# k-flouris/cmf

Measured on AMD Instinct MI355X. Metric: log-density evals/sec (JtJ-cholesky path), MNIST D=784 d=64 bs=512, higher is better.
Workload: dtype f32 (3x3 tangent convs as bf16x3 split MFMA, fp32 accumulate); 1 GPU; C3: MNIST-shaped (1,28,28) uint8-range + U[0,1) noise, non-square flow d=64, cholesky J^T J log-det + g_ij off-diagonal L1 + reconstruction, eval/no_grad; per_gpu_batch=512, global_batch=512, D=784, latent_dimension=64, parallelism=dp1

## Files before the change

### cmf_amd/_lib.py

```python
import ctypes as C
import os
import threading

_HERE = os.path.dirname(os.path.abspath(__file__))
LIB_PATH = os.path.join(_HERE, "libcmf_amd.so")

F_NONE, F_RELU, F_TANH, F_RAW, F_SELF_RELU, F_RELU_BITS = 0, 1, 2, 3, 4, 5
O_NONE, O_TANH, O_STANH = 0, 1, 2

_fp = C.c_void_p
_ll = C.c_longlong
_i = C.c_int
_f = C.c_float
_d = C.c_double


class ConvTangentArgs(C.Structure):
    _fields_ = [("x", _fp), ("x_np", _ll), ("x_ci", _ll), ("x_px", _ll),
                ("f", _fp), ("f_np", _ll), ("f_ci", _ll), ("f_px", _ll), ("fmode", _i),
                ("w", _fp),
                ("y", _fp), ("y_np", _ll), ("y_co", _ll), ("y_px", _ll),
                ("r", _fp), ("r_np", _ll), ("r_co", _ll), ("r_px", _ll),
                ("np", _i), ("cin", _i), ("cout", _i), ("H", _i), ("W", _i), ("nc", _i), ("taps", _i),
                ("bias", _fp), ("f_group", _i), ("x_sl", _ll), ("y_sl", _ll), ("r_sl", _ll),
                ("fo", _fp), ("fo_np", _ll), ("fo_co", _ll), ("fo_px", _ll), ("fomode", _i),
                ("mask_out", _fp), ("mask_np", _ll), ("amax_in", _fp), ("amax_out", _fp), ("live", _i),
                ("ymask", _fp), ("ymask_np", _ll)]


class ConvPrimalArgs(C.Structure):
    _fields_ = [("x", _fp), ("x_b", _ll), ("x_c", _ll), ("x_px", _ll),
                ("f", _fp), ("f_c", _ll), ("f_px", _ll), ("imode", _i),
                ("w", _fp), ("bias", _fp), ("sw", _fp), ("sb", _fp),
                ("y", _fp), ("y_b", _ll), ("y_c", _ll), ("y_px", _ll),
                ("g", _fp),
                ("r", _fp), ("r_b", _ll), ("r_c", _ll), ("r_px", _ll),
                ("omode", _i),
                ("B", _i), ("cin", _i), ("cout", _i), ("H", _i), ("W", _i), ("taps", _i)]


MLP_MAX_LAYERS = 8
WGRAD_MAX_BATCH = 16


class MlpCouplerArgs(C.Structure):
    _fields_ = [("z", _fp), ("z_b", _ll), ("t", _fp), ("t_f", _ll), ("w", _fp),
                ("zi", _fp), ("si", _fp), ("ti", _fp), ("n_mod", _i),
                ("B", _i), ("cin", _i), ("chan_off", _i), ("chan_step", _i), ("n_layers", _i),
                ("width", _i * (MLP_MAX_LAYERS + 1)), ("w_off", _ll * MLP_MAX_LAYERS), ("decode", _i), ("lj", _fp), ("ncols", _i)]


SIGNATURES = {
    "cmf_version": (C.c_char_p, []),
    "cmf_pack_weight": (_i, [_fp, _fp, _i, _i, _i, _i, C.POINTER(_ll), _fp]),
    "cmf_pack_weights_batched": (_i, [_fp, _i, _fp]),
    "cmf_conv_tangent": (_i, [C.POINTER(ConvTangentArgs), _fp]),
    "cmf_pack_weight_bf16x3": (_i, [_fp, _fp, _i, _i, C.POINTER(_ll), _fp]),
    "cmf_pack_weight_bf16x3_t": (_i, [_fp, _fp, _i, _i, _i, C.POINTER(_ll), _fp]),
    "cmf_conv_tangent_bf16x3": (_i, [C.POINTER(ConvTangentArgs), _fp]),
    "cmf_pack_weight_f16x3": (_i, [_fp, _fp, _i, _i, _i, C.POINTER(_ll), _fp]),
    "cmf_conv_tangent_f16x3": (_i, [C.POINTER(ConvTangentArgs), _fp]),
    "cmf_conv_tangent_f16x3_item": (_i, [C.POINTER(ConvTangentArgs), _i, _fp]),
    "cmf_absmax": (_i, [_fp, _ll, _fp, _fp]),
    "cmf_conv_tangent_wgrad_ws": (_ll, [C.POINTER(ConvTangentArgs)]),
    "cmf_conv_tangent_wgrad": (_i, [C.POINTER(ConvTangentArgs), _fp, _fp, _fp, _ll, _fp]),
    "cmf_conv_tangent_wgrad_bf16x3": (_i, [C.POINTER(ConvTangentArgs), _fp, _fp, _fp, _ll, _fp]),
    "cmf_conv_tangent_wgrad_bf16x3_batched": (_i, [C.POINTER(ConvTangentArgs), _i, C.POINTER(_fp), C.POINTER(_fp), C.POINTER(_fp), _fp, _ll, _fp]),
    "cmf_primal_regroup": (_i, [_fp, _fp, _i, _ll, _i, _fp]),
    "cmf_conv_primal": (_i, [C.POINTER(ConvPrimalArgs), _fp]),
    "cmf_acl_primal": (_i, [_fp, _ll, _fp, _ll, _fp, _fp, _fp, _i, _i, _i, _fp, _fp]),
    "cmf_acl_tangent": (_i, [_fp, _ll, _ll, _fp, _ll, _ll, _i, _fp, _ll, _fp, _ll, _fp, _fp, _fp, _fp, _i, _i, _fp]),
    "cmf_acl_cotangent": (_i, [_fp, _ll, _ll, _fp, _ll, _ll, _i, _fp, _ll, _fp, _ll, _fp, _fp, _fp, _fp, _i, _i, _fp]),
    "cmf_acl_primal_backward": (_i, [_fp, _ll, _fp, _ll, _fp, _ll, _fp, _fp, _fp, _fp, _i, _i, _i, _fp, _fp]),
    "cmf_acl_cross_terms": (_i, [_fp, _ll, _ll, _fp, _ll, _ll, _fp, _ll, _ll, _i, _fp, _ll, _fp, _ll, _fp, _fp, _fp, _fp, _i, _i,
                            _fp, _fp, _fp, _fp]),
    "cmf_gather_primal": (_i, [_fp, _ll, _fp, _ll, _fp, _i, _i, _fp]),
    "cmf_gather_tangent": (_i, [_fp, _ll, _ll, _fp, _ll, _ll, _fp, _i, _i, _i, _fp]),
    "cmf_seed_tangent": (_i, [_fp, _ll, _ll, _fp, _i, _i, _fp, _i, _i, _i, _fp]),
    "cmf_gram_cholesky": (_i, [_fp, _ll, _ll, _i, _i, _i, _i, _fp, _fp, _fp, _fp, _fp, _fp, _fp]),
    "cmf_cholesky_retry": (_i, [_fp, _i, _i, _i, _f, _fp, _fp, _fp, _fp, _fp]),
# ... 131 lines not shown
```

### cmf_amd/csrc/common.h

```cpp
#pragma once
#include <hip/hip_runtime.h>
#include "cmf_amd.h"

typedef float f32x4 __attribute__((ext_vector_type(4)));

#define CMF_LAUNCH_CHECK()                         \
  do {                                             \
    hipError_t e_ = hipGetLastError();             \
    if (e_ != hipSuccess) return (int)e_;          \
  } while (0)

hipError_t cmf_set_dynamic_lds(const void* fn, int bytes);
int cmf_device_cus();

static inline int cmf_ceil_div(long long a, long long b) { return (int)((a + b - 1) / b); }

__device__ __forceinline__ float wave_sum(float v) {
#pragma unroll
  for (int o = 32; o > 0; o >>= 1) v += __shfl_xor(v, o, 64);
  return v;
}

__device__ __forceinline__ float block_sum(float v, float* red) {
  v = wave_sum(v);
  const int w = threadIdx.x >> 6, nw = (blockDim.x + 63) >> 6;
  __syncthreads();
  if ((threadIdx.x & 63) == 0) red[w] = v;
  __syncthreads();
  float t = 0.f;
  for (int i = 0; i < nw; ++i) t += red[i];
  return t;
}

int cmf_wide_gram_cholesky(const float* t, long long t_b, long long t_r, int n_rows, int d, int B, float* jtj, float* logdet,
                           float* l1_off, float* l1_diag, int* info, int* fail, hipStream_t s);
int cmf_wide_cholesky_retry(float* jtj, int d, int B, int attempt, float eps, float* logdet, float* l1_diag, int* info, int* fail,
                            hipStream_t s);
int cmf_wide_gram_backward(const float* t, long long t_b, long long t_r, int n_rows, int nc, int d, int B, const float* jtj,
                           const float* g_logdet, const float* g_l1off, const float* g_l1diag, float* dt, long long dt_b,
                           long long dt_r, float* ws, hipStream_t s);
int cmf_wide_gram_backward_matrix(const float* t, long long t_b, long long t_r, int n_rows, int nc, int d, int B, const float* m,
                                  float* dt, long long dt_b, long long dt_r, hipStream_t s);
int cmf_wide_hutch_cg(const float* jtj, const float* eps, int d, int S, int B, int max_iter, int min_iter, float tol, float* u,
                      float* w, float* val, int* iters, hipStream_t s);
int cmf_wide_hutch_cotangent(const float* u, const float* eps, const float* w, int d, int S, int B, const float* g_val,
                             const float* g_off, const float* g_diag, float* M, hipStream_t s);
```

### cmf_amd/csrc/conv_tangent_bf16x3.hip

```cpp
#include <cstdlib>
#include <type_traits>
#include "common.h"

#ifdef CMF_DBG_STAMP
__device__ unsigned long long cmf_dbg_stamps[3][64][4];
extern "C" int cmf_debug_read_stamps(void* out) {
  return (int)hipMemcpyFromSymbol(out, HIP_SYMBOL(cmf_dbg_stamps), sizeof(cmf_dbg_stamps));
}
#define STAMP(role, g, k)                                                                        \
  do {                                                                                            \
    if (blockIdx.x == 0 && (g) < 64 && lane == 0 && wave == ((role) == 1 ? 4 : 0)) {                   \
      unsigned long long t_;                                                                      \
      asm volatile("s_memtime %0\n\ts_waitcnt lgkmcnt(0)" : "=s"(t_)::"memory");                  \
      cmf_dbg_stamps[role][g][k] = t_;                                                            \
    }                                                                                             \
  } while (0)
__device__ unsigned long long cmf_dbg_wg_span[1024][2];
extern "C" int cmf_debug_read_wg_span(void* out) {
  return (int)hipMemcpyFromSymbol(out, HIP_SYMBOL(cmf_dbg_wg_span), sizeof(cmf_dbg_wg_span));
}
#define SPAN(k)                                                                                   \
  do {                                                                                            \
    if (lane == 0 && wave == 0 && blockIdx.x < 1024) {                                            \
      unsigned long long t_;                                                                      \
// ... 1027 lines not shown
}

template <int PXW>
int launch_cot(const cmf_conv_tangent_args& a, hipStream_t s) {
  if (a.ymask) return a.fmode == CMF_F_RELU ? launch<4, PXW, 6>(a, s) : launch<4, PXW, 7>(a, s);
  if (a.fmode == CMF_F_SELF_RELU) return (a.cout > 32) ? launch<4, PXW, 2>(a, s) : launch<2, PXW, 2>(a, s);
  if (a.fmode == CMF_F_RELU) return (a.cout > 32) ? launch<4, PXW, 1>(a, s) : launch<2, PXW, 1>(a, s);
  if (a.fmode == CMF_F_RELU_BITS) return (a.cout > 32) ? launch<4, PXW, 3>(a, s) : launch<2, PXW, 3>(a, s);
  if (a.fmode == CMF_F_NONE && a.fomode == CMF_F_RELU_BITS && a.r) {
    return launch<4, PXW, 5>(a, s);
  }
  if (a.fmode == CMF_F_NONE) return (a.cout > 32) ? launch<4, PXW, 4>(a, s) : launch<2, PXW, 4>(a, s);
  return (a.cout > 32) ? launch<4, PXW, 0>(a, s) : launch<2, PXW, 0>(a, s);
}

inline bool fits_int(long long v) { return v >= 0 && v < (1LL << 29); }

}

extern "C" int cmf_pack_weight_bf16x3_t(const float* w, void* out, int cout, int cin, int transpose, long long* out_bytes, void* stream);
extern "C" int cmf_pack_weight_bf16x3(const float* w, void* out, int cout, int cin, long long* out_bytes, void* stream) {
  return cmf_pack_weight_bf16x3_t(w, out, cout, cin, 0, out_bytes, stream);
}
extern "C" int cmf_pack_weight_bf16x3_t(const float* w, void* out, int cout, int cin, int transpose, long long* out_bytes, void* stream) {
  if (cout <= 0 || cin <= 0 || cin % 8) return CMF_EINVAL;
  const long long total = (long long)((cout + 63) / 64) * (cin / 8) * 2 * 3 * 4 * 4 * 16 * 8;
  if (out_bytes) *out_bytes = total * 2;
  if (!out) return 0;
  if (!w) return CMF_EINVAL;
  hipLaunchKernelGGL(pack_weight_bf16x3_kernel, dim3((unsigned)((total + 255) / 256)), dim3(256), 0, (hipStream_t)stream,
                     w, (unsigned short*)out, cout, cin, total, transpose ? 1 : 0, 0);
  CMF_LAUNCH_CHECK();
  return 0;
}

extern "C" int cmf_pack_weight_f16x3(const float* w, void* out, int cout, int cin, int transpose, long long* out_bytes, void* stream) {
  if (cout <= 0 || cin <= 0 || cin % 8) return CMF_EINVAL;
  const long long total = (long long)((cout + 63) / 64) * (cin / 8) * 2 * 3 * 4 * 4 * 16 * 8;
  if (out_bytes) *out_bytes = total * 2 + 16;
  if (!out) return 0;
  if (!w || (uintptr_t)out % 16) return CMF_EINVAL;
  hipLaunchKernelGGL(pack_f16_scale_kernel, dim3(1), dim3(1024), 0, (hipStream_t)stream, w, (long long)cout * cin * 9,
                     reinterpret_cast<float*>((unsigned short*)out + total));
  CMF_LAUNCH_CHECK();
  hipLaunchKernelGGL(pack_weight_bf16x3_kernel, dim3((unsigned)((total + 255) / 256)), dim3(256), 0, (hipStream_t)stream,
                     w, (unsigned short*)out, cout, cin, total, transpose ? 1 : 0, 1);
  CMF_LAUNCH_CHECK();
  return 0;
}

extern "C" int cmf_conv_tangent_bf16x3(const cmf_conv_tangent_args* ap, void* stream) {
  if (!ap) return CMF_EINVAL;
  const cmf_conv_tangent_args& a = *ap;
  if (!a.x || !a.w || !a.y || a.np <= 0 || a.cin <= 0 || a.cout <= 0 || a.H <= 0 || a.W <= 0) return CMF_EINVAL;
  if (a.taps != 9 || a.cin % 32 || a.nc <= 0 || a.nc % 16) return CMF_EINVAL;
  if (a.fmode < CMF_F_NONE || a.fmode > CMF_F_RELU_BITS) return CMF_EINVAL;
  if (a.fmode != CMF_F_SELF_RELU && a.fmode != CMF_F_NONE && !a.f) return CMF_EINVAL;
  if (a.mask_out) return CMF_EINVAL;
  if (a.fo) {
    const bool inplace = a.r == a.y && a.r_np == a.y_np && a.r_co == a.y_co && a.r_px == a.y_px && a.r_sl == a.y_sl;
    if (a.fmode != CMF_F_NONE || a.fomode != CMF_F_RELU_BITS || (a.r && !inplace) || a.cout % 64) return CMF_EINVAL;
    if (a.r && a.bias) return CMF_EINVAL;
    if (a.fo_np % 4 || (uintptr_t)a.fo % 4 || a.fo_np < (long long)a.H * a.W * (a.cout / 8)) return CMF_EINVAL;
  }
  if (a.fmode == CMF_F_RELU_BITS && a.f_np < (long long)a.H * a.W * (a.cin / 8)) return CMF_EINVAL;
  if (a.ymask) {
    if ((a.fmode != CMF_F_RELU && a.fmode != CMF_F_RELU_BITS) || a.cout % 64 || a.live || a.fo || a.r || a.bias) return CMF_EINVAL;
    if (a.ymask_np % 4 || (uintptr_t)a.ymask % 4 || a.ymask_np < (long long)a.H * a.W * (a.cout / 8)) return CMF_EINVAL;
  }
  if ((a.x_np | a.x_ci | a.x_px | a.x_sl | a.y_sl | a.r_sl) % 4 || ((uintptr_t)a.x % 16) || ((uintptr_t)a.w % 16)) return CMF_EINVAL;
  if ((a.y_np | a.y_co | a.y_px) % 4 || ((uintptr_t)a.y % 16)) return CMF_EINVAL;
  if (a.r && ((a.r_np | a.r_co | a.r_px) % 4 || ((uintptr_t)a.r % 16))) return CMF_EINVAL;
  const long long HW = (long long)a.H * a.W;
  if (!fits_int((a.cin + 8) * a.x_ci + HW * a.x_px + a.nc) || !fits_int((a.cin + 8) * a.f_ci + HW * a.f_px) ||
      !fits_int((a.cout + 64) * a.y_co + HW * a.y_px + a.nc + 64) ||
      (a.r && !fits_int((a.cout + 64) * a.r_co + HW * a.r_px + a.nc)) ||
      HW > (1 << 24))
    return CMF_ERANGE;
  hipStream_t s = (hipStream_t)stream;
  const bool t14 = a.W % 14 == 0 && a.H % 2 == 0, t8 = a.W % 8 == 0 && a.H % 4 == 0;
  if (!(t14 || t8) || !(a.cout % 64 == 0 || a.cout == 32)) return CMF_EINVAL;
  if (a.bias && a.cout > 64) return CMF_EINVAL;
  if (a.live) {
    if (a.live < 0 || a.live > 2 || (a.fmode != CMF_F_RELU && a.fmode != CMF_F_RELU_BITS) || a.fo || a.bias || a.cout % 64 || a.W % 2)
      return CMF_EINVAL;
    if (a.fmode == CMF_F_RELU) return t14 ? launch<4, 7, 1, false, false, true>(a, s) : launch<4, 4, 1, false, false, true>(a, s);
    return t14 ? launch<4, 7, 3, false, false, true>(a, s) : launch<4, 4, 3, false, false, true>(a, s);
  }
  if (a.fmode == CMF_F_NONE && !a.fo) {
    cmf_conv_tangent_args b = a;
    b.fo = a.x;
    b.fo_np = 0;
    b.fomode = CMF_F_NONE;
    return t14 ? launch_cot<7>(b, s) : launch_cot<4>(b, s);
  }
  return t14 ? launch_cot<7>(a, s) : launch_cot<4>(a, s);
}

extern "C" int cmf_conv_tangent_f16x3(const cmf_conv_tangent_args* ap, void* stream) {
  return cmf_conv_tangent_f16x3_item(ap, 0, stream);
}

extern "C" int cmf_conv_tangent_f16x3_item(const cmf_conv_tangent_args* ap, int item_channels, void* stream) {
  if (!ap || (item_channels != 0 && item_channels != 32 && item_channels != 64)) return CMF_EINVAL;
  const cmf_conv_tangent_args& a = *ap;
  if (!a.x || !a.w || !a.y || a.np <= 0 || a.cin <= 0 || a.cout <= 0 || a.H <= 0 || a.W <= 0) return CMF_EINVAL;
// ... 34 lines not shown
```

### cmf_amd/engine.py

```python
import ctypes as C
import threading

import numpy as np
import torch
import torch.nn as nn

from . import _lib
from ._lib import (F_NONE, F_RELU, F_TANH, F_RAW, F_SELF_RELU, F_RELU_BITS, O_NONE, O_TANH, O_STANH, ConvPrimalArgs,
                   ConvTangentArgs)


def _stream():
    return C.c_void_p(torch.cuda.current_stream().cuda_stream)


def _p(t):
    return None if t is None else C.c_void_p(t.data_ptr())


def require_gpu(t, what="input"):
    if not t.is_cuda:
        raise RuntimeError(f"cmf_amd: {what} is on {t.device}; the log-density path runs only through the HIP "
                           "kernels on an AMD GPU (there is no CPU fallback)")
    if t.dtype != torch.float32:
# ... 247 lines not shown
                continue
            if not isinstance(w, nn.Parameter):
                continue
            todo.append((key, w, ver, out, taps))
        if not todo:
            return
        desc = np.dtype([("w", "<u8"), ("out", "<u8"), ("total", "<i8"), ("cout", "<i4"), ("cin", "<i4"), ("taps", "<i4"),
                         ("transpose", "<i4"), ("kind", "<i4"), ("reserved", "<i4")])
        sig = tuple((key, w.data_ptr(), out.data_ptr()) for key, w, ver, out, taps in todo)
        cached = self._tables.get(device)
        if cached is not None and cached[0] == sig:
            table = cached[1]
        else:
            arr = np.zeros(len(todo), dtype=desc)
            for i, (key, w, ver, out, taps) in enumerate(todo):
                _, transpose, bf16x3 = key
                cout, cin = int(w.shape[0]), int(w.shape[1])
                if bf16x3 and transpose:
                    cout, cin = cin, cout
                total = out.numel() * out.element_size()
                total = (total - 16) // 2 if bf16x3 == 2 else total // (2 if bf16x3 else 4)
                arr[i] = (w.data_ptr(), out.data_ptr(), total, cout, cin, taps, int(transpose), int(bf16x3), 0)
            table = torch.from_numpy(arr.view(np.uint8).copy()).to(device)
            self._tables[device] = (sig, table)
        _lib.check(_lib.load().cmf_pack_weights_batched(_p(table), len(todo), _stream()), "cmf_pack_weights_batched")
        order = self._mark()
        for key, w, ver, out, taps in todo:
            self._store[key] = (self._store[key][0], ver[:4] + (self.generation,), out, taps, order)


PACKS = _PackCache()




def conv_primal(x_ptr_t, x_off, x_b, x_c, x_px, weight, taps, bias, y, y_b, y_c, y_px, B, cin, cout, H, W,
                imode=F_NONE, mask=None, f_c=0, f_px=0, omode=O_NONE, sw=None, sb=None, g=None, res=None):
    lib = _lib.load()
    a = ConvPrimalArgs()
    a.x = C.c_void_p(x_ptr_t.data_ptr() + 4 * int(x_off)); a.x_b, a.x_c, a.x_px = int(x_b), int(x_c), int(x_px)
    a.f = _p(mask); a.f_c, a.f_px = int(f_c), int(f_px); a.imode = imode
    a.w = _p(PACKS.get(weight, taps)); a.bias = _p(bias); a.sw = _p(sw); a.sb = _p(sb)
    a.y = _p(y); a.y_b, a.y_c, a.y_px = int(y_b), int(y_c), int(y_px)
    a.g = _p(g)
    a.r = _p(res); a.r_b, a.r_c, a.r_px = int(y_b), int(y_c), int(y_px)
    a.omode = omode
    a.B, a.cin, a.cout, a.H, a.W, a.taps = int(B), int(cin), int(cout), int(H), int(W), int(taps)
    _lib.check(lib.cmf_conv_primal(C.byref(a), _stream()), "cmf_conv_primal")


def conv_tangent(x_t, x_off, x_np, x_ci, x_px, weight, taps, y_t, y_np, y_co, y_px, np_, cin, cout, H, W, nc,
                 fmode=F_NONE, f=None, f_np=0, f_ci=0, f_px=0, res_t=None, transpose=False, bias=None, f_group=1,
                 x_sl=16, y_sl=16, precision=None, y_off=0, res_off=0, fo=None, fo_np=0, fo_co=0, fo_px=0, fomode=F_NONE,
                 mask_out=None, mask_np=0, amax_in=None, amax_out=None, item_channels=0, live=0, res_np=None, ymask=None):
    lib = _lib.load()
    a = ConvTangentArgs()
    a.x = C.c_void_p(x_t.data_ptr() + 4 * int(x_off)); a.x_np, a.x_ci, a.x_px = int(x_np), int(x_ci), int(x_px)
    a.f = _p(f); a.f_np, a.f_ci, a.f_px = int(f_np), int(f_ci), int(f_px); a.fmode = fmode
    obits = isinstance(fo, BitMask)
    inplace = res_t is not None and res_t.data_ptr() == y_t.data_ptr() and int(res_off) == int(y_off)
    precision = precision or cfg().tangent
    split = (precision == "bf16x3" and _shape_ok_bf16x3(taps, cin, W, transpose, H, cout)
             and not (bias is not None and cout > 64)
             and ((fmode != F_NONE and fo is None) or
                  (fmode == F_NONE and (fo is None or (obits and (res_t is None or inplace) and cout % 64 == 0)))))
    pbwd = fmode == F_NONE and fo is not None and not obits and fomode == F_SELF_RELU
    f16 = (precision == "f16x3" and cout % 64 == 0 and _shape_ok_bf16x3(taps, cin, W, transpose, H, cout)
           and not (bias is not None and cout > 64)
           and ((fmode == F_SELF_RELU and fo is None and not transpose) or (pbwd and bias is None and mask_out is None)))
    assert not obits or split, "bit-mask output factors are applied by the split-precision kernel only"
    if obits:
        fo, fo_np, fo_co, fo_px, fomode = fo.data, fo.np_bytes, 0, 0, F_RELU_BITS
    a.w = _p(PACKS.get(weight, taps, transpose, bf16x3="f16x3" if f16 else split))
    a.y = C.c_void_p(y_t.data_ptr() + 4 * int(y_off)); a.y_np, a.y_co, a.y_px = int(y_np), int(y_co), int(y_px)
    a.r = None if res_t is None else C.c_void_p(res_t.data_ptr() + 4 * int(res_off))
    a.r_np, a.r_co, a.r_px = int(y_np if res_np is None else res_np), int(y_co), int(y_px)
    a.fo = _p(fo); a.fo_np, a.fo_co, a.fo_px, a.fomode = int(fo_np), int(fo_co), int(fo_px), int(fomode)
    a.mask_out = _p(mask_out); a.mask_np = int(mask_np)
    assert not (fmode == F_RELU_BITS and not split), "bit-mask factors are read by the split-precision kernel only"
    assert not (mask_out is not None and split), "sign bits are written by the fp32 and the fp16-split kernels only"
    a.amax_in, a.amax_out = (_p(amax_in), _p(amax_out)) if f16 else (None, None)
    a.live = int(live)
    assert not live or split, "checkerboard output is the split-precision kernel's"
    assert ymask is None or split, "the store filter is the split-precision kernel's"
    if ymask is not None:
        a.ymask, a.ymask_np = _p(ymask.data), int(ymask.np_bytes)
    a.np, a.cin, a.cout, a.H, a.W, a.nc, a.taps = int(np_), int(cin), int(cout), int(H), int(W), int(nc), int(taps)
    a.bias = _p(bias); a.f_group = int(f_group)
    a.x_sl, a.y_sl, a.r_sl = int(x_sl), int(y_sl), int(y_sl)
    fn, what = ((lib.cmf_conv_tangent_f16x3, "cmf_conv_tangent_f16x3") if f16 else
                (lib.cmf_conv_tangent_bf16x3, "cmf_conv_tangent_bf16x3") if split else (lib.cmf_conv_tangent, "cmf_conv_tangent"))
    launch = lambda: _lib.check(fn(C.byref(a), _stream()), what)
    if f16 and item_channels:
        launch = lambda: _lib.check(lib.cmf_conv_tangent_f16x3_item(C.byref(a), int(item_channels), _stream()), "cmf_conv_tangent_f16x3_item")
    if fmode == F_SELF_RELU and not f16 and _lib.tracing():
        run = launch

        def launch():
            with _lib.role("primal"):
                run()
    TIMER = _timer()
    if TIMER is None:
        return launch()
    px_in = float(H) * W * nc * np_
    px = px_in * (0.5 if live else 1.0)
    TIMER.wrap(f"conv_tangent_t{taps}_ci{cin}_co{cout}" + ("_primal" if fmode == F_SELF_RELU else "_primal_bwd" if pbwd else "_live" if live else ""),
               2.0 * cin * cout * taps * px,
               4.0 * (px_in * cin + px * (cout + (cout if res_t is not None else 0))), launch)


_WGRAD_WS = {}


def conv_tangent_wgrad(x_t, x_off, x_np, x_ci, x_px, gy_t, gy_off, y_np, y_co, y_px, dw, taps, np_, cin, cout, H, W, nc,
                       fmode=F_NONE, f=None, f_np=0, f_ci=0, f_px=0, f_group=1, x_sl=16, y_sl=16, precision=None):
    lib = _lib.load()
    assert dw.dtype == torch.float32 and dw.is_contiguous() and dw.numel() == cout * cin * taps
    a = ConvTangentArgs()
    a.x = C.c_void_p(x_t.data_ptr() + 4 * int(x_off)); a.x_np, a.x_ci, a.x_px = int(x_np), int(x_ci), int(x_px)
    fbits = isinstance(f, BitMask)
    if fbits:
        f, f_np, f_ci, f_px, fmode = f.data, f.np_bytes, 0, 0, F_RELU_BITS
    a.f = _p(f); a.f_np, a.f_ci, a.f_px = int(f_np), int(f_ci), int(f_px); a.fmode = fmode
    a.y_np, a.y_co, a.y_px = int(y_np), int(y_co), int(y_px)
    a.np, a.cin, a.cout, a.H, a.W, a.nc, a.taps = int(np_), int(cin), int(cout), int(H), int(W), int(nc), int(taps)
    a.f_group = int(f_group)
    a.x_sl, a.y_sl = int(x_sl), int(y_sl)
    need = int(lib.cmf_conv_tangent_wgrad_ws(C.byref(a)))
    key = (x_t.device, torch.cuda.current_stream().cuda_stream)
    ws = _WGRAD_WS.get(key)
    if ws is None or ws.numel() * 4 < need:
        ws = _WGRAD_WS[key] = torch.empty(need // 4, dtype=torch.float32, device=x_t.device)
    gy = C.c_void_p(gy_t.data_ptr() + 4 * int(gy_off))
    split = ((precision or cfg().tangent) == "bf16x3" and taps == 9 and cin % 64 == 0 and cout % 64 == 0 and nc % 32 == 0
             and fmode in (F_NONE, F_RELU, F_SELF_RELU, F_RELU_BITS) and f_group <= 1)
    assert not fbits or split, "bit-mask factors are read by the split-precision weight-gradient kernel only"
    fn, what = (lib.cmf_conv_tangent_wgrad_bf16x3, "cmf_conv_tangent_wgrad_bf16x3") if split else \
               (lib.cmf_conv_tangent_wgrad, "cmf_conv_tangent_wgrad")
    launch = lambda: _lib.check(fn(C.byref(a), gy, _p(dw), _p(ws), need, _stream()), what)
    TIMER = _timer()
    if TIMER is None:
        return launch()
    px = float(H) * W * nc * np_
    TIMER.wrap(f"conv_wgrad_t{taps}_ci{cin}_co{cout}" + ("_primal" if fmode == F_SELF_RELU else ""), 2.0 * cin * cout * taps * px,
               4.0 * px * (cin + cout), launch)


def conv_tangent_wgrad_batched(xs, gys, dws, x_np, x_ci, x_px, y_np, y_co, y_px, np_, cin, cout, H, W, nc, fmode=F_NONE, x_sl=16, y_sl=16):
    lib = _lib.load()
    n = len(xs)
    assert n == len(gys) == len(dws) and 1 <= n <= _lib.WGRAD_MAX_BATCH and fmode in (F_NONE, F_SELF_RELU)
    assert cin % 64 == 0 and cout % 64 == 0 and nc % 32 == 0
    a = ConvTangentArgs()
    a.x = _p(xs[0]); a.x_np, a.x_ci, a.x_px = int(x_np), int(x_ci), int(x_px)
    a.fmode = fmode
    a.y_np, a.y_co, a.y_px = int(y_np), int(y_co), int(y_px)
    a.np, a.cin, a.cout, a.H, a.W, a.nc, a.taps = int(np_), int(cin), int(cout), int(H), int(W), int(nc), 9
    a.f_group = 1
    a.x_sl, a.y_sl = int(x_sl), int(y_sl)
    need = int(lib.cmf_conv_tangent_wgrad_ws(C.byref(a)))
    key = (xs[0].device, torch.cuda.current_stream().cuda_stream)
# ... 769 lines not shown
    a = primal_regroup(a0, True)
    acts, masks = [a], []
    rng = None
    if prec == "f16x3":
        rng = torch.zeros(2 * len(blocks) + 1, dtype=torch.float32, device=dev)
        absmax(a, rng[0:1])
    ax = lambda i: dict(amax_in=rng[i:i + 1], amax_out=rng[i + 1:i + 2]) if rng is not None else {}
    for k, blk in enumerate(blocks):
        c1, a2 = new(), new()
        m1, m2 = (BitMask(B, HW, hid, dev), BitMask(B, HW, hid, dev)) if bits else (None, None)
        mo = lambda m: dict(mask_out=m.data, mask_np=m.np_bytes) if m is not None else {}
        conv_tangent(a, 0, *pn, blk.conv1.weight, 9, c1, *pn, G, hid, hid, H, W, 16, fmode=F_SELF_RELU, bias=blk.conv1.bias,
                     precision=prec, **mo(m1), **ax(2 * k))
        conv_tangent(c1, 0, *pn, blk.conv2.weight, 9, a2, *pn, G, hid, hid, H, W, 16, fmode=F_SELF_RELU, bias=blk.conv2.bias,
                     res_t=a, precision=prec, **mo(m2), **ax(2 * k + 1))
        acts += [c1, a2]
        masks += [m1, m2]
        a = a2
    yg = torch.empty(G * cout * HW * 16, dtype=torch.float32, device=dev)
    gg = torch.empty_like(yg)
    conv_primal(a, 0, hid * HW * 16, HW * 16, 1, convf.weight, 1, convf.bias, yg, cout * HW * 16, HW * 16, 1, G, hid, cout,
                1, HW * 16, imode=F_RELU, omode=O_STANH, sw=net.weights.detach().reshape(-1), sb=net.bias.detach().reshape(-1),
                g=gg)
    y = primal_regroup(yg.view(G, -1), False).view(B, cout, H, W)
    g = primal_regroup(gg.view(G, -1), False).view(B, cout, H, W)
    if not need_acts:
        return y, g, None
    std_of = lambda t: primal_regroup(t.view(G, -1), False).view(B, hid, H, W)
    if train:
        out = ActList([a0] + masks[:-1] + [std_of(acts[-1])] if bits else [a0] + [std_of(t) for t in acts[1:]])
        out.grouped = acts
        return y, g, out
    if bits:
        return y, g, [a0] + masks[:-1] + [std_of(acts[-1])]
    return y, g, [a0] + [std_of(t) for t in acts[1:]]


def _view_rows(T, view):
    if T.layout == "panel":
        HW = view.geom.HW
        rows = T.data[: T.B * T.N * T.nc].view(T.B, T.N // HW, HW * T.nc)[:, view.chan_off::view.chan_step][:, :view.cin]
        out = Tangent(T.B, view.cin * HW, T.nc, "panel", T.data.device)
    else:
        rows = T.data[: T.B * T.N * T.nc].view(T.N, T.B * T.nc)[view.chan_off::view.chan_step][:view.cin]
        out = Tangent(T.B, view.cin, T.nc, "fmajor", T.data.device)
    out.data.view(rows.shape).copy_(rows)
    return out


CHECKERBOARD_TAIL = True

SKIP_DEAD_ROWS = True


def net_tangent(net, T, view, acts, transpose_packs=False, save=None):
    geo, B, nc, dev = view.geom, T.B, T.nc, T.data.device
    if save is not None:
        save.append(_view_rows(T, view))
    if net.kind == "resnet":
        conv0, blocks, convf = _resnet_parts(net)
        hid, cout, H, W, HW = conv0.out_channels, convf.out_channels, geo.H, geo.W, geo.HW
        new = lambda c: Tangent(B, c * HW, nc, "panel", dev)
        pn = lambda c: (c * HW * nc, HW * nc, nc)
        hd = (hid * HW * nc, 16, hid * nc)
        hsl = hid * 16
        h = new(hid)
        conv_tangent(T.data, view.chan_off * HW * nc, T.t_b, view.chan_step * HW * nc, nc, conv0.weight, 9, h.data, *hd,
                     B, view.cin, hid, H, W, nc, fmode=F_RAW if view.mask is not None else F_NONE, f=view.mask, f_np=0,
                     f_ci=HW, f_px=1, y_sl=hsl)
        fg = getattr(acts, "f_group", 1)
        fs = dict(f_np=hid * HW * fg, f_ci=HW * fg, f_px=fg, f_group=fg)
        fk = lambda t: dict(fmode=F_RELU_BITS, f=t.data, f_np=t.np_bytes) if isinstance(t, BitMask) else dict(fmode=F_RELU, f=t, **fs)
        u, h2 = new(hid), new(hid)
        compact = (CHECKERBOARD_TAIL and view.live is not None and save is None and fg == 1 and len(blocks) > 0 and hid % 64 == 0
                   and W % 2 == 0 and _use_bf16x3(9, hid, W, False, H, hid))
        filt = SKIP_DEAD_ROWS and save is None and hid % 64 == 0 and _use_bf16x3(9, hid, W, False, H, hid)
        for k, blk in enumerate(blocks):
            a_in, c1 = acts[2 * k], acts[2 * k + 1]
            conv_tangent(h.data, 0, *hd, blk.conv1.weight, 9, u.data, *hd, B, hid, hid, H, W, nc, x_sl=hsl, y_sl=hsl, **fk(a_in),
                         ymask=c1 if filt and isinstance(c1, BitMask) else None)
            if compact and k + 1 == len(blocks):
                HWc = HW // 2
                hc = Tangent(B, hid * HWc, nc, "panel", dev)
                conv_tangent(u.data, 0, *hd, blk.conv2.weight, 9, hc.data, hid * HWc * nc, 16, hid * nc, B, hid, hid, H, W, nc,
                             res_t=h.data, res_np=hd[0], x_sl=hsl, y_sl=hsl, live=view.live["parity"], **fk(c1))
                a_last = gather_primal(acts[-1], view.live["act_idx"], hid * HWc)
                yt = Tangent(B, cout * HWc, nc, "panel", dev)
                conv_tangent(hc.data, 0, hid * HWc * nc, 16, hid * nc, convf.weight, 1, yt.data, cout * HWc * nc, HWc * nc, nc, B, hid,
                             cout, H, W // 2, nc, fmode=F_RELU, f=a_last, x_sl=hsl, f_np=hid * HWc, f_ci=HWc, f_px=1)
                yt.compact = True
                return yt
            conv_tangent(u.data, 0, *hd, blk.conv2.weight, 9, h2.data, *hd, B, hid, hid, H, W, nc, res_t=h.data, x_sl=hsl,
                         y_sl=hsl, **fk(c1))
            if save is not None:
                save += [h, u]
                h, u, h2 = h2, new(hid), new(hid)
            else:
                h, h2 = h2, h
        if save is not None:
            save.append(h)
        yt = new(cout)
        conv_tangent(h.data, 0, *hd, convf.weight, 1, yt.data, *pn(cout), B, hid, cout, H, W, nc, fmode=F_RELU,
                     f=acts[-1], x_sl=hsl, **fs)
        return yt
    lins = [m for m in net if isinstance(m, nn.Linear)]
    x_t, x_off, x_ci, cin = T.data, view.chan_off * B * nc, view.chan_step * B * nc, view.cin
    fmode, f, f_px = F_NONE, None, 0
    out = None
    for i, lin in enumerate(lins):
        out = Tangent(B, lin.out_features, nc, "fmajor", dev)
        conv_tangent(x_t, x_off, 0, x_ci, nc, lin.weight, 1, out.data, 0, B * nc, nc, 1, cin, lin.out_features, 1, B, nc,
                     fmode=fmode, f=f, f_np=0, f_ci=1, f_px=f_px)
        if i < len(acts):
            fmode, f, f_px = F_TANH, acts[i], lin.out_features
        x_t, x_off, x_ci, cin = out.data, 0, B * nc, lin.out_features
        if save is not None and i + 1 < len(lins):
            save.append(out)
    return out


class GradPool(dict):

    def __init__(self, params, device):
        super().__init__()
        n = sum((p.numel() + 3) // 4 * 4 for p in params)
        self._pool = torch.zeros(max(n, 4), dtype=torch.float32, device=device)
        self._used = 0

    def zeros_for(self, weight):
        n = weight.numel()
        if self._used + n > self._pool.numel():
            return torch.zeros_like(weight, dtype=torch.float32).contiguous()
        g = self._pool[self._used:self._used + n].view(weight.shape)
# ... 219 lines not shown
```

### include/cmf_amd.h

```cpp
#ifndef CMF_AMD_H
#define CMF_AMD_H

#ifdef __cplusplus
extern "C" {
#endif

#define CMF_EINVAL (-1)
#define CMF_ERANGE (-2)

#define CMF_F_NONE 0
#define CMF_F_RELU 1
#define CMF_F_TANH 2
#define CMF_F_RAW  3
#define CMF_F_SELF_RELU 4
#define CMF_F_RELU_BITS 5

#define CMF_O_NONE  0
#define CMF_O_TANH  1
#define CMF_O_STANH 2

const char* cmf_version(void);

int cmf_pack_weight(const float* w, float* out, int cout, int cin, int taps, int transpose,
                    long long* out_floats, void* stream);

typedef struct {
  const float* w; void* out; long long total;
  int cout, cin, taps, transpose, kind, reserved;
} cmf_pack_desc;
int cmf_pack_weights_batched(const cmf_pack_desc* table, int n, void* stream);

typedef struct {
  const float* x; long long x_np, x_ci, x_px;
  const float* f; long long f_np, f_ci, f_px;
  int fmode;
  const float* w;
  float* y;       long long y_np, y_co, y_px;
  const float* r; long long r_np, r_co, r_px;
  int np, cin, cout, H, W, nc, taps;
  const float* bias;
  int f_group;
  long long x_sl, y_sl, r_sl;
  const float* fo; long long fo_np, fo_co, fo_px; int fomode;
  void* mask_out; long long mask_np;
  const float* amax_in; float* amax_out;
  int live;
  const void* ymask; long long ymask_np;
} cmf_conv_tangent_args;
int cmf_conv_tangent(const cmf_conv_tangent_args* a, void* stream);

int cmf_pack_weight_bf16x3(const float* w, void* out, int cout, int cin, long long* out_bytes, void* stream);
int cmf_pack_weight_bf16x3_t(const float* w, void* out, int cout, int cin, int transpose, long long* out_bytes, void* stream);
int cmf_conv_tangent_bf16x3(const cmf_conv_tangent_args* a, void* stream);

int cmf_pack_weight_f16x3(const float* w, void* out, int cout, int cin, int transpose, long long* out_bytes, void* stream);
int cmf_conv_tangent_f16x3(const cmf_conv_tangent_args* a, void* stream);
int cmf_conv_tangent_f16x3_item(const cmf_conv_tangent_args* a, int item_channels, void* stream);
int cmf_absmax(const float* x, long long n, float* out, void* stream);

long long cmf_conv_tangent_wgrad_ws(const cmf_conv_tangent_args* a);
int cmf_conv_tangent_wgrad(const cmf_conv_tangent_args* a, const float* gy, float* dw, float* ws, long long ws_bytes,
                           void* stream);
int cmf_conv_tangent_wgrad_bf16x3(const cmf_conv_tangent_args* a, const float* gy, float* dw, float* ws, long long ws_bytes,
                                  void* stream);
#define CMF_WGRAD_MAX_BATCH 16
int cmf_conv_tangent_wgrad_bf16x3_batched(const cmf_conv_tangent_args* a, int nprob, const float* const* x, const float* const* gy,
                                          float* const* dw, float* ws, long long ws_bytes, void* stream);

typedef struct {
  const float* x; long long x_b, x_c, x_px;
  const float* f; long long f_c, f_px;
  int imode;
  const float* w; const float* bias;
  const float* sw; const float* sb;
  float* y;       long long y_b, y_c, y_px;
  float* g;
  const float* r; long long r_b, r_c, r_px;
  int omode;
  int B, cin, cout, H, W, taps;
} cmf_conv_primal_args;
int cmf_conv_primal(const cmf_conv_primal_args* a, void* stream);

int cmf_primal_regroup(const float* in, float* out, int B, long long N, int to_grouped, void* stream);

int cmf_acl_primal(float* z, long long z_b, const float* y, long long y_b, const int* zi, const int* si,
                   const int* ti, int n_mod, int B, int decode, float* lj, void* stream);
int cmf_acl_cotangent(float* c, long long c_b, long long c_r, float* yc, long long yc_b, long long yc_r, int nc,
                      const float* z, long long z_b, const float* y, long long y_b, const float* g, const int* zi,
                      const int* si, const int* ti, int n_mod, int B, void* stream);
int cmf_acl_primal_backward(float* dx, long long dx_b, const float* z, long long z_b, const float* y, long long y_b, float* dy,
                            const int* zi, const int* si, const int* ti, int n_mod, int B, int decode, const float* dlj,
                            void* stream);
int cmf_acl_cross_terms(const float* c, long long c_b, long long c_r, const float* v, long long v_b, long long v_r,
                        const float* yt, long long yt_b, long long yt_r, int nc, const float* z, long long z_b,
                        const float* y, long long y_b, const float* g, const int* zi, const int* si, const int* ti,
                        int n_mod, int B, float* dz, float* dy, float* dg, void* stream);
int cmf_acl_tangent(float* t, long long t_b, long long t_r, const float* yt, long long yt_b, long long yt_r,
                    int nc, const float* z, long long z_b, const float* y, long long y_b, const float* g,
                    const int* zi, const int* si, const int* ti, int n_mod, int B, void* stream);

// ... 105 lines not shown
```

Baseline: 1449 evals/s.

## Fold final residual 3x3 tangent conv and 1x1 head into one kernel

Adds a dedicated kernel for the last residual block that composes the 1x1 output head (gated by its ReLU activation) with the 3x3 conv2 weights, giving per-pixel effective coefficients. Each output pixel's small cout tangent is then computed straight from the 3x3 neighbourhood of the input tangent plus the residual, so the hid-channel intermediate tangent is never written and the separate 1x1 conv launch is skipped. The cost is fp32 FMA work without MFMA, and the path only covers hid=64, cout<=8 and ReLU-bitmask inputs. Extra shape and stride checks guard the path, and the original path stays as the fallback.

```diff
diff --git a/cmf_amd/_lib.py b/cmf_amd/_lib.py
--- a/cmf_amd/_lib.py
+++ b/cmf_amd/_lib.py
@@ -25,7 +25,9 @@
                 ("bias", _fp), ("f_group", _i), ("x_sl", _ll), ("y_sl", _ll), ("r_sl", _ll),
                 ("fo", _fp), ("fo_np", _ll), ("fo_co", _ll), ("fo_px", _ll), ("fomode", _i),
                 ("mask_out", _fp), ("mask_np", _ll), ("amax_in", _fp), ("amax_out", _fp), ("live", _i),
-                ("ymask", _fp), ("ymask_np", _ll)]
+                ("ymask", _fp), ("ymask_np", _ll),
+                ("head_w", _fp), ("head_cout", _i), ("head_a", _fp), ("head_a_np", _ll), ("head_a_c", _ll), ("head_a_px", _ll),
+                ("head_y", _fp), ("head_y_np", _ll), ("head_y_co", _ll), ("head_y_px", _ll)]
 
 
 class ConvPrimalArgs(C.Structure):
diff --git a/cmf_amd/csrc/common.h b/cmf_amd/csrc/common.h
--- a/cmf_amd/csrc/common.h
+++ b/cmf_amd/csrc/common.h
@@ -32,6 +32,8 @@
   return t;
 }
 
+int cmf_conv_head(const cmf_conv_tangent_args& a, hipStream_t s);
+
 int cmf_wide_gram_cholesky(const float* t, long long t_b, long long t_r, int n_rows, int d, int B, float* jtj, float* logdet,
                            float* l1_off, float* l1_diag, int* info, int* fail, hipStream_t s);
 int cmf_wide_cholesky_retry(float* jtj, int d, int B, int attempt, float eps, float* logdet, float* l1_diag, int* info, int* fail,
diff --git a/cmf_amd/csrc/conv_head.hip b/cmf_amd/csrc/conv_head.hip
--- /dev/null
+++ b/cmf_amd/csrc/conv_head.hip
@@ -0,0 +1,202 @@
+#include <stdint.h>
+
+#include "common.h"
+
+namespace {
+
+constexpr int HID = 64, KJ = HID * 9, NT = 192, ACC = 16;
+constexpr int SLICE = HID * 16;
+
+__device__ __forceinline__ int out_pixel(int po, int W, int live) {
+  if (!live) return po;
+  const int wh = W >> 1, row = po / wh, k = po - row * wh;
+  return row * W + 2 * k + ((row + live - 1) & 1);
+}
+
+template <int CP>
+__global__ __launch_bounds__(NT, CP == 8 ? 2 : 3) void conv_head_kernel(cmf_conv_tangent_args a, int n_out, int tiles_per_sample, int ntiles) {
+  constexpr int P = ACC / CP;
+  __shared__ __attribute__((aligned(16))) float Es[P * KJ * CP];
+  __shared__ __attribute__((aligned(16))) float Gs[HID * ACC];
+  __shared__ unsigned long long um[P * 9];
+  __shared__ unsigned long long alv[P];
+  __shared__ int pixs[P];
+
+  const int per = (ntiles + 7) >> 3;
+  const int item = (int)(blockIdx.x & 7) * per + (int)(blockIdx.x >> 3);
+  if (item >= ntiles) return;
+  const int b = item / tiles_per_sample, p0 = (item - b * tiles_per_sample) * P;
+  const int cnt = n_out - p0 < P ? n_out - p0 : P;
+  const int tid = threadIdx.x, lane = tid & 63, wv = tid >> 6;
+  const int H = a.H, W = a.W, cout = a.head_cout;
+
+  if (tid < P * 9) {
+    const int p = tid / 9, tap = tid - p * 9;
+    unsigned long long m = 0;
+    if (p < cnt) {
+      const int pix = out_pixel(p0 + p, W, a.live);
+      const int r = pix / W + tap / 3 - 1, c = pix % W + tap % 3 - 1;
+      if (r >= 0 && r < H && c >= 0 && c < W)
+        m = *reinterpret_cast<const unsigned long long*>(reinterpret_cast<const unsigned char*>(a.f) + (long long)b * a.f_np +
+                                                         (long long)(r * W + c) * (HID / 8));
+    }
+    um[tid] = m;
+  }
+  for (int p = wv; p < P; p += NT / 64) {
+    const int pix = p < cnt ? out_pixel(p0 + p, W, a.live) : 0;
+    bool on = false;
+    if (p < cnt) on = a.head_a[(long long)b * a.head_a_np + (long long)lane * a.head_a_c + (long long)pix * a.head_a_px] > 0.f;
+    const unsigned long long bal = __ballot(on);
+    if (lane == 0) {
+      alv[p] = bal;
+      pixs[p] = pix;
+    }
+#pragma unroll
+    for (int o = 0; o < CP; ++o) Gs[(lane * P + p) * CP + o] = (on && o < cout) ? a.head_w[o * HID + lane] : 0.f;
+  }
+  __syncthreads();
+
+  {
+    static_assert(3 * NT == KJ, "three (ci, tap) pairs per thread");
+    float acc[3][ACC];
+#pragma unroll
+    for (int r = 0; r < 3; ++r)
+#pragma unroll
+      for (int i = 0; i < ACC; ++i) acc[r][i] = 0.f;
+#pragma unroll 2
+    for (int c = 0; c < HID; ++c) {
+      float w[3];
+#pragma unroll
+      for (int r = 0; r < 3; ++r) w[r] = a.w[c * KJ + tid + r * NT];
+#pragma unroll
+      for (int i = 0; i < ACC / 4; ++i) {
+        const f32x4 g = *reinterpret_cast<const f32x4*>(&Gs[c * ACC + 4 * i]);
+#pragma unroll
+        for (int r = 0; r < 3; ++r)
+#pragma unroll
+          for (int k = 0; k < 4; ++k) acc[r][4 * i + k] = fmaf(g[k], w[r], acc[r][4 * i + k]);
+      }
+    }
+#pragma unroll
+    for (int r = 0; r < 3; ++r)
+#pragma unroll
+      for (int p = 0; p < P; ++p)
+#pragma unroll
+        for (int o = 0; o < CP; ++o) Es[(p * KJ + tid + r * NT) * CP + o] = acc[r][p * CP + o];
+  }
+  __syncthreads();
+
+  const int nsl = a.nc >> 4, cl = lane >> 2;
+  const f32x4 zero = {0.f, 0.f, 0.f, 0.f};
+  for (int unit = wv; unit < nsl * P; unit += NT / 64) {
+    const int sl = unit / P, p = unit - sl * P;
+    if (p >= cnt) continue;
+    const int pix = pixs[p];
+    const float* hb = a.r + (long long)b * a.r_np + (long long)pix * a.r_px + sl * SLICE + lane * 4;
+    const float* ub = a.x + (long long)b * a.x_np + sl * SLICE + lane * 4;
+    f32x4 acc[CP];
+#pragma unroll
+    for (int o = 0; o < CP; ++o) acc[o] = zero;
+
+    auto load4 = [&](f32x4* v, const float* src, unsigned long long m) {
+#pragma unroll
+      for (int ch = 0; ch < 4; ++ch) {
+        v[ch] = zero;
+        if ((m >> (ch * 16 + cl)) & 1) v[ch] = *reinterpret_cast<const f32x4*>(src + ch * 256);
+      }
+    };
+    auto load_row = [&](f32x4* v, int ty) {
+#pragma unroll
+      for (int tx = 0; tx < 3; ++tx)
+        load4(v + 4 * tx, ub + (long long)(pix + (ty - 1) * W + (tx - 1)) * a.x_px, um[p * 9 + ty * 3 + tx]);
+    };
+    auto fma4 = [&](const f32x4* v, const float* coef, int stride) {
+#pragma unroll
+      for (int ch = 0; ch < 4; ++ch) {
+        const float* e4 = static_cast<const float*>(__builtin_assume_aligned(coef + ch * stride, CP < 4 ? 8 : 16));
+#pragma unroll
+        for (int o = 0; o < CP; ++o) {
+          const float e = e4[o];
+#pragma unroll
+          for (int k = 0; k < 4; ++k) acc[o][k] = fmaf(e, v[ch][k], acc[o][k]);
+        }
+      }
+    };
+    auto fma_row = [&](const f32x4* v, int ty) {
+#pragma unroll
+      for (int tx = 0; tx < 3; ++tx) fma4(v + 4 * tx, &Es[(p * KJ + cl * 9 + ty * 3 + tx) * CP], 16 * 9 * CP);
+    };
+    {
+      f32x4 vh[4], v[12];
+      load4(vh, hb, alv[p]);
+      load_row(v, 0);
+      fma4(vh, &Gs[(cl * P + p) * CP], 16 * P * CP);
+      fma_row(v, 0);
+    }
+#pragma unroll 1
+    for (int ty = 1; ty < 3; ++ty) {
+      f32x4 v[12];
+      load_row(v, ty);
+      fma_row(v, ty);
+    }
+
+    constexpr int N = 4 * CP;
+    float val[N];
+#pragma unroll
+    for (int o = 0; o < CP; ++o)
+#pragma unroll
+      for (int k = 0; k < 4; ++k) val[4 * o + k] = acc[o][k];
+#pragma unroll
+    for (int s = 0; s < 4; ++s) {
+      const int off = 32 >> s, n = N >> s;
+      if (n >= 2) {
+        const bool hi = lane & off;
+#pragma unroll
+        for (int i = 0; i < n / 2; ++i) {
+          const float mine = hi ? val[n / 2 + i] : val[i], send = hi ? val[i] : val[n / 2 + i];
+          val[i] = mine + __shfl_xor(send, off, 64);
+        }
+      } else {
+        val[0] += __shfl_xor(val[0], off, 64);
+      }
+    }
+    float* yb = a.head_y + (long long)b * a.head_y_np + (long long)(p0 + p) * a.head_y_px + sl * 16 + (lane & 3) * 4;
+    constexpr int KEEP = N >= 16 ? N / 16 : 1;
+#pragma unroll
+    for (int i = 0; i < KEEP; ++i) {
+      const int idx = ((cl * N) >> 4) + i, o = idx >> 2;
+      if (o < cout && (N >= 16 || !(lane & 4))) yb[(long long)o * a.head_y_co + (idx & 3)] = val[i];
+    }
+  }
+}
+
+template <int CP>
+int launch(const cmf_conv_tangent_args& a, hipStream_t s) {
+  constexpr int P = ACC / CP;
+  const int n_out = a.live ? a.H * a.W / 2 : a.H * a.W;
+  const long long tiles = (n_out + P - 1) / P, ntiles = tiles * a.np;
+  if (ntiles > 0x7ffffff0LL) return CMF_ERANGE;
+  const int grid = 8 * (int)((ntiles + 7) / 8);
+  hipLaunchKernelGGL(conv_head_kernel<CP>, dim3(grid), dim3(NT), 0, s, a, n_out, (int)tiles, (int)ntiles);
+  CMF_LAUNCH_CHECK();
+  return 0;
+}
+
+}
+
+int cmf_conv_head(const cmf_conv_tangent_args& a, hipStream_t s) {
+  if (!a.x || !a.w || !a.f || !a.r || !a.head_w || !a.head_a || !a.head_y) return CMF_EINVAL;
+  if (a.fmode != CMF_F_RELU_BITS || a.taps != 9 || a.cin != HID || a.cout != HID) return CMF_EINVAL;
+  if (a.head_cout < 1 || a.head_cout > 8 || a.np <= 0 || a.H <= 0 || a.W <= 0 || a.nc <= 0 || a.nc % 16) return CMF_EINVAL;
+  if (a.bias || a.fo || a.ymask || a.mask_out || a.live < 0 || a.live > 2 || (a.live && a.W % 2)) return CMF_EINVAL;
+  if (!((a.W % 14 == 0 && a.H % 2 == 0) || (a.W % 8 == 0 && a.H % 4 == 0))) return CMF_EINVAL;
+  const long long HW = (long long)a.H * a.W;
+  if (HW > (1 << 24)) return CMF_ERANGE;
+  if (a.x_ci != 16 || a.x_sl != SLICE || a.r_co != 16 || a.r_sl != SLICE) return CMF_EINVAL;
+  if ((a.x_np | a.x_px | a.r_np | a.r_px | a.head_y_np | a.head_y_co | a.head_y_px) % 4) return CMF_EINVAL;
+  if (a.x_px < (long long)HID * a.nc || a.r_px < (long long)HID * a.nc || a.head_y_px < a.nc) return CMF_EINVAL;
+  if ((uintptr_t)a.x % 16 || (uintptr_t)a.r % 16 || (uintptr_t)a.head_y % 16 || (uintptr_t)a.w % 4 || (uintptr_t)a.head_w % 4) return CMF_EINVAL;
+  if ((uintptr_t)a.f % 8 || a.f_np % 8 || a.f_np < HW * (HID / 8)) return CMF_EINVAL;
+  const int cp = a.head_cout <= 2 ? 2 : a.head_cout <= 4 ? 4 : 8;
+  return cp == 2 ? launch<2>(a, s) : cp == 4 ? launch<4>(a, s) : launch<8>(a, s);
+}
diff --git a/cmf_amd/csrc/conv_tangent_bf16x3.hip b/cmf_amd/csrc/conv_tangent_bf16x3.hip
--- a/cmf_amd/csrc/conv_tangent_bf16x3.hip
+++ b/cmf_amd/csrc/conv_tangent_bf16x3.hip
@@ -1103,6 +1103,7 @@
 extern "C" int cmf_conv_tangent_bf16x3(const cmf_conv_tangent_args* ap, void* stream) {
   if (!ap) return CMF_EINVAL;
   const cmf_conv_tangent_args& a = *ap;
+  if (a.head_w) return cmf_conv_head(a, (hipStream_t)stream);
   if (!a.x || !a.w || !a.y || a.np <= 0 || a.cin <= 0 || a.cout <= 0 || a.H <= 0 || a.W <= 0) return CMF_EINVAL;
   if (a.taps != 9 || a.cin % 32 || a.nc <= 0 || a.nc % 16) return CMF_EINVAL;
   if (a.fmode < CMF_F_NONE || a.fmode > CMF_F_RELU_BITS) return CMF_EINVAL;
diff --git a/cmf_amd/engine.py b/cmf_amd/engine.py
--- a/cmf_amd/engine.py
+++ b/cmf_amd/engine.py
@@ -323,9 +323,14 @@
 def conv_tangent(x_t, x_off, x_np, x_ci, x_px, weight, taps, y_t, y_np, y_co, y_px, np_, cin, cout, H, W, nc,
                  fmode=F_NONE, f=None, f_np=0, f_ci=0, f_px=0, res_t=None, transpose=False, bias=None, f_group=1,
                  x_sl=16, y_sl=16, precision=None, y_off=0, res_off=0, fo=None, fo_np=0, fo_co=0, fo_px=0, fomode=F_NONE,
-                 mask_out=None, mask_np=0, amax_in=None, amax_out=None, item_channels=0, live=0, res_np=None, ymask=None):
+                 mask_out=None, mask_np=0, amax_in=None, amax_out=None, item_channels=0, live=0, res_np=None, ymask=None, head=None):
     lib = _lib.load()
     a = ConvTangentArgs()
+    if head is not None:
+        assert (precision or cfg().tangent) == "bf16x3" and not transpose and bias is None and fo is None and ymask is None \
+            and mask_out is None, "the folded head replaces the split-precision forward conv + 1x1 conv only"
+        return _conv_tangent_head(lib, a, x_t, x_off, x_np, x_ci, x_px, weight, taps, y_t, y_np, y_co, y_px, np_, cin, cout, H, W, nc,
+                                  fmode, f, f_np, res_t, res_off, res_np, x_sl, y_off, live, head)
     a.x = C.c_void_p(x_t.data_ptr() + 4 * int(x_off)); a.x_np, a.x_ci, a.x_px = int(x_np), int(x_ci), int(x_px)
     a.f = _p(f); a.f_np, a.f_ci, a.f_px = int(f_np), int(f_ci), int(f_px); a.fmode = fmode
     obits = isinstance(fo, BitMask)
@@ -378,6 +383,31 @@
     TIMER.wrap(f"conv_tangent_t{taps}_ci{cin}_co{cout}" + ("_primal" if fmode == F_SELF_RELU else "_primal_bwd" if pbwd else "_live" if live else ""),
                2.0 * cin * cout * taps * px,
                4.0 * (px_in * cin + px * (cout + (cout if res_t is not None else 0))), launch)
+
+
+def _conv_tangent_head(lib, a, x_t, x_off, x_np, x_ci, x_px, weight, taps, y_t, y_np, y_co, y_px, np_, cin, cout, H, W, nc, fmode, f,
+                       f_np, res_t, res_off, res_np, x_sl, y_off, live, head):
+    wf, act = head["weight"], head["act"]
+    hc = int(wf.shape[0])
+    w2, wf = weight.detach(), wf.detach().reshape(hc, -1)
+    assert w2.is_contiguous() and wf.is_contiguous() and act.is_contiguous() and w2.dtype == wf.dtype == act.dtype == torch.float32
+    a.x = C.c_void_p(x_t.data_ptr() + 4 * int(x_off)); a.x_np, a.x_ci, a.x_px, a.x_sl = int(x_np), int(x_ci), int(x_px), int(x_sl)
+    a.f = _p(f); a.f_np = int(f_np); a.fmode = int(fmode)
+    a.w = _p(w2)
+    a.r = None if res_t is None else C.c_void_p(res_t.data_ptr() + 4 * int(res_off))
+    a.r_np, a.r_co, a.r_px, a.r_sl = int(x_np if res_np is None else res_np), int(x_ci), int(x_px), int(x_sl)
+    a.np, a.cin, a.cout, a.H, a.W, a.nc, a.taps, a.live = int(np_), int(cin), int(cout), int(H), int(W), int(nc), int(taps), int(live)
+    a.head_w, a.head_cout = _p(wf), hc
+    a.head_a = _p(act); a.head_a_np, a.head_a_c, a.head_a_px = int(cin) * H * W, H * W, 1
+    a.head_y = C.c_void_p(y_t.data_ptr() + 4 * int(y_off)); a.head_y_np, a.head_y_co, a.head_y_px = int(y_np), int(y_co), int(y_px)
+    launch = lambda: _lib.check(lib.cmf_conv_tangent_bf16x3(C.byref(a), _stream()), "cmf_conv_tangent_bf16x3")
+    TIMER = _timer()
+    if TIMER is None:
+        return launch()
+    px_out = float(H) * W * np_ * (0.5 if live else 1.0)
+    TIMER.wrap(f"conv_tangent_t{taps}_ci{cin}_co{cout}" + ("_live" if live else ""),
+               2.0 * hc * px_out * (cin * taps * cout + (cin * taps + cout) * nc),
+               4.0 * (float(H) * W * np_ * nc * cin + px_out * (nc * cout + cout + nc * hc)), launch)
 
 
 _WGRAD_WS = {}
@@ -1253,6 +1283,8 @@
 
 SKIP_DEAD_ROWS = True
 
+FOLD_HEAD = True
+
 
 def net_tangent(net, T, view, acts, transpose_packs=False, save=None):
     geo, B, nc, dev = view.geom, T.B, T.nc, T.data.device
@@ -1276,10 +1308,21 @@
         compact = (CHECKERBOARD_TAIL and view.live is not None and save is None and fg == 1 and len(blocks) > 0 and hid % 64 == 0
                    and W % 2 == 0 and _use_bf16x3(9, hid, W, False, H, hid))
         filt = SKIP_DEAD_ROWS and save is None and hid % 64 == 0 and _use_bf16x3(9, hid, W, False, H, hid)
+        fold = (FOLD_HEAD and view.live is not None and save is None and fg == 1 and len(blocks) > 0 and hid == 64 and cout <= 8 and nc % 16 == 0
+                and isinstance(acts[2 * len(blocks) - 1], BitMask) and _use_bf16x3(9, hid, W, False, H, hid))
         for k, blk in enumerate(blocks):
             a_in, c1 = acts[2 * k], acts[2 * k + 1]
             conv_tangent(h.data, 0, *hd, blk.conv1.weight, 9, u.data, *hd, B, hid, hid, H, W, nc, x_sl=hsl, y_sl=hsl, **fk(a_in),
                          ymask=c1 if filt and isinstance(c1, BitMask) else None)
+            if fold and k + 1 == len(blocks):
+                HWo = HW // 2 if compact else HW
+                yt = Tangent(B, cout * HWo, nc, "panel", dev)
+                conv_tangent(u.data, 0, *hd, blk.conv2.weight, 9, yt.data, cout * HWo * nc, HWo * nc, nc, B, hid, hid, H, W, nc,
+                             res_t=h.data, res_np=hd[0], x_sl=hsl, live=view.live["parity"] if compact else 0,
+                             head=dict(weight=convf.weight, act=acts[-1]), **fk(c1))
+                if compact:
+                    yt.compact = True
+                return yt
             if compact and k + 1 == len(blocks):
                 HWc = HW // 2
                 hc = Tangent(B, hid * HWc, nc, "panel", dev)
diff --git a/include/cmf_amd.h b/include/cmf_amd.h
--- a/include/cmf_amd.h
+++ b/include/cmf_amd.h
@@ -46,6 +46,9 @@
   const float* amax_in; float* amax_out;
   int live;
   const void* ymask; long long ymask_np;
+  const float* head_w; int head_cout;
+  const float* head_a; long long head_a_np, head_a_c, head_a_px;
+  float* head_y; long long head_y_np, head_y_co, head_y_px;
 } cmf_conv_tangent_args;
 int cmf_conv_tangent(const cmf_conv_tangent_args* a, void* stream);
 
```

Result: faster. 1468 evals/s (median of 6 runs) (+1.3%).
